# o1-labs/proof-systems

Hardware: AMD Instinct MI355X
Metric: MSM Mscalar/s at 2^20 (Vesta) (higher is better)
Workload: dtype u29x9 / u32x8 (255-bit Montgomery integers); 1 GPU; msm_2^20_vesta_srs; points_per_gpu=1048576, points_total=1048576, bases=SRS::<Vesta>::create, scalars=uniform 254-bit, seed 1234+rank, parallelism=point-range x1, world_size_seen=1

## Files before the change

### include/kimchi_hip.h

```cpp
#ifndef KIMCHI_HIP_H
#define KIMCHI_HIP_H

#include <stddef.h>
#include <stdint.h>

#ifdef __cplusplus
extern "C" {
#endif

#define KH_OK 0
#define KH_E_INVALID (-1)
#define KH_E_DEVICE (-2)
#define KH_E_NOTFOUND (-3)
#define KH_E_NOMEM (-4)

#define KH_CURVE_VESTA 0
#define KH_CURVE_PALLAS 1
#define KH_FIELD_FP 0
#define KH_FIELD_FQ 1
#define KH_BASIS_G (-1)

typedef struct kh_srs kh_srs_t;
typedef struct kh_sponge kh_sponge_t;

// ... 258 lines not shown
int kh_msm_submit_host(kh_srs_t *srs, int basis, unsigned chunk, size_t offset,
                       const uint64_t *scalars , size_t n, size_t k, int scalars_are_montgomery,
                       uint64_t *ticket);
int kh_ntt_dev(int field, uint64_t *data_dev, unsigned log2_n, int inverse, size_t batch);
int kh_lde_dev(int field, const uint64_t *coeffs_dev, unsigned log2_n, unsigned log2_blowup,
               uint64_t *out_dev, size_t batch);
int kh_coset_ntt_dev(int field, const uint64_t *coeffs_dev, unsigned log2_n, const uint64_t shift[4], uint64_t *out_dev, size_t batch);
int kh_sync(void);

int kh_last_timings(const char **names, float *ms, int cap);
uint64_t kh_counter(const char *name);

int kh_debug_field_op(int field, int op, const uint64_t *a, const uint64_t *b, uint64_t *out, size_t n);
int kh_debug_rebase_points(kh_srs_t *srs, const uint64_t *coef, size_t Q, uint64_t *out_xy, uint32_t *out_fail);
int kh_debug_glv_split(int scalar_field, const uint64_t *scalars, size_t n, uint32_t *out);
int kh_debug_point_op(int curve, int op, const uint64_t *p_xy, const uint8_t *p_inf,
                      const uint64_t *q_xy, const uint8_t *q_inf,
                      uint64_t *out_xy, uint8_t *out_inf, size_t n);

typedef struct kh_comm kh_comm_t;
#define KH_COMM_ID_BYTES 128
int kh_comm_unique_id(uint8_t id[128]);
int kh_comm_init(int world_size, int rank, const uint8_t id[128], kh_comm_t **out);
void kh_comm_free(kh_comm_t *comm);
int kh_comm_world_size(const kh_comm_t *comm);
int kh_comm_rank(const kh_comm_t *comm);
int kh_comm_allgather_points(kh_comm_t *comm, const uint64_t *xy, const uint8_t *inf, size_t k, uint64_t *out_xy, uint8_t *out_inf);
int kh_msm_allreduce(kh_comm_t *comm, kh_srs_t *shard, const uint64_t *scalars, size_t n, int scalars_are_montgomery, uint64_t out_xy[8],
                     uint8_t *out_is_inf);

// ... 151 lines not shown
```

### proof_systems_amd/csrc/common.hpp

```cpp
#pragma once
#include <hip/hip_runtime.h>
#include <stdarg.h>
#include <stdint.h>
#include <stdio.h>
#include <atomic>
#include <chrono>
#include <condition_variable>
#include <initializer_list>
#include <map>
#include <memory>
#include <mutex>
#include <set>
#include <string>
#include <thread>
#include <vector>

#include "../../include/kimchi_hip.h"

namespace kh {

void set_error(const char* fmt, ...);

#define KH_HIP(expr)                                                                         \
    do {                                                                                     \
// ... 92 lines not shown
        ws_b29, ws_a1, ws_l2, ws_a2, ws_xlist;
    void* pinned = nullptr; size_t pinned_cap = 0;
    hipEvent_t done = nullptr;
    bool busy = false;
    std::thread::id owner;
    uint64_t ticket = 0;
    MsmJob job;
    std::shared_ptr<std::atomic<int>> handle_jobs;
    volatile uint32_t* host_abort = nullptr;
    volatile uint32_t* spread_abort = nullptr;
    bool flag_unavailable = false;
    bool pinned_coherent = false;
    volatile uint32_t* done_flag = nullptr;
    DevBuf ws_done;
    uint32_t done_expect = 0;
};
static constexpr int MSM_SLOTS = 4;

struct Context {
    std::mutex mu;
    std::condition_variable cv;
    int sync_inflight = 0;
    std::multiset<std::thread::id> blocked_owners;
    int device = -1;
    bool ready = false;
    hipStream_t stream = nullptr;
    bool main_dirty = false;
    hipEvent_t order_ev = nullptr;
    int num_cus = 256;
    size_t lds_per_cu = (size_t)160 << 10, lds_per_block = (size_t)64 << 10;
    bool fused_disabled = false;
    PhaseTimer timer;
    std::vector<std::pair<const char*, float>> last;
    MsmSlot slot[MSM_SLOTS];
    uint64_t next_ticket = 1;
    std::chrono::steady_clock::time_point last_sync_msm_arrival{};
    DevBuf ws_ntt_a, ws_ntt_b;
    void* pinned = nullptr; size_t pinned_cap = 0;
    char* stage = nullptr; size_t stage_cap = 0, stage_cur = 0;
    int stage_upload(void* dst_dev, std::initializer_list<std::pair<const void*, size_t>> parts);
    void mark_async() { if (hipEventRecord(order_ev, stream) == hipSuccess) main_dirty = true; }
    std::mutex scratch_mu;
    std::map<std::string, DevBuf> scratch_bufs;
    std::set<std::string> done_flags;
    DevBuf& scratch(const char* name) { std::lock_guard<std::mutex> lk(scratch_mu); return scratch_bufs[name]; }
    bool once(const char* name) { std::lock_guard<std::mutex> lk(scratch_mu); return done_flags.insert(name).second; }
    void trim_scratch() { std::lock_guard<std::mutex> lk(scratch_mu); for (auto& kv : scratch_bufs) kv.second.release(); }
};
static constexpr int KH_MAX_DEVICES = 16;

// ... 23 lines not shown
```

### proof_systems_amd/csrc/debug_api.cpp

```cpp
#include "api_internal.hpp"

using namespace kh;

extern "C" {

int kh_debug_rebase_points(kh_srs_t* srs, const uint64_t* coef, size_t Q, uint64_t* out_xy, uint32_t* out_fail) {
    KH_ON_DEVICE_OF(srs);
    KH_REQUIRE(srs && coef && out_xy && out_fail, "kh_debug_rebase_points: null argument");
    KH_REQUIRE(srs->g_precomp_c == 16, "the handle has no c = 16 window tables");
    KH_REQUIRE(Q >= 1 && srs->n % Q == 0 && (srs->n / Q) % 64 == 0, "Q = %zu must divide the SRS size %zu into a multiple of 64", Q, srs->n);
    int rc = ensure_init(); if (rc) return rc;
    Context& C = ctx();
    std::lock_guard<std::mutex> lk(C.mu);
    const size_t N = srs->n / Q;
    DevBuf B, part, lists, out, dcoef, fail, scratch;
    if ((rc = B.reserve(rebase_bucket_bytes(N))) || (rc = part.reserve(rebase_part_bytes(N))) || (rc = lists.reserve(rebase_list_bytes(Q))) || (rc = out.reserve(N * 64)) ||
        (rc = dcoef.reserve(Q * 32)) || (rc = fail.reserve(64)) || (rc = scratch.reserve(N * 128))) return rc;
    KH_HIP(hipMemcpyAsync(dcoef.p, coef, Q * 32, hipMemcpyHostToDevice, C.stream));
    KH_HIP(hipMemsetAsync(fail.p, 0, 64, C.stream));
    if ((rc = rebase_points(C.stream, srs->curve, dcoef.as<uint64_t>(), Q, srs->g.p, srs->g_stride, N, B.p, part.p, lists.p))) return rc;
    if ((rc = rebase_tables(C.stream, srs->curve, part.p, N, nullptr, 0, 256, scratch.p, out.p, fail.as<uint32_t>()))) return rc;
    KH_HIP(hipMemcpyAsync(out_xy, out.p, N * 64, hipMemcpyDeviceToHost, C.stream));
    KH_HIP(hipMemcpyAsync(out_fail, fail.p, 4, hipMemcpyDeviceToHost, C.stream));
    KH_HIP(hipStreamSynchronize(C.stream));
    return KH_OK;
}
int kh_debug_glv_split(int scalar_field, const uint64_t* scalars, size_t n, uint32_t* out) {
    KH_REQUIRE(scalar_field == KH_FIELD_FP || scalar_field == KH_FIELD_FQ, "unknown field id %d", scalar_field);
    KH_REQUIRE(scalars && out, "kh_debug_glv_split: null argument");
    int rc = ensure_init(); if (rc) return rc;
    if (n == 0) return KH_OK;
    Context& C = ctx();
    std::lock_guard<std::mutex> lk(C.mu);
    DevBuf din, dout;
    if ((rc = din.reserve(n * 32)) || (rc = dout.reserve(n * 40))) return rc;
    KH_HIP(hipMemcpyAsync(din.p, scalars, n * 32, hipMemcpyHostToDevice, C.stream));
    if ((rc = msm_debug_glv_split(C.stream, scalar_field, din.as<uint64_t>(), n, dout.as<uint32_t>()))) return rc;
    KH_HIP(hipMemcpyAsync(out, dout.p, n * 40, hipMemcpyDeviceToHost, C.stream));
    KH_HIP(hipStreamSynchronize(C.stream));
    return KH_OK;
}
int kh_debug_field_op(int field, int op, const uint64_t* a, const uint64_t* b, uint64_t* out, size_t n) {
    KH_REQUIRE(a && out, "null argument");
    int rc = ensure_init(); if (rc) return rc;
    if (n == 0) return KH_OK;
    Context& C = ctx();
    std::lock_guard<std::mutex> lk(C.mu);
    void *da = nullptr, *db = nullptr, *dout = nullptr;
    KH_HIP(hipMalloc(&da, n * 32)); KH_HIP(hipMalloc(&dout, n * 32));
    KH_HIP(hipMemcpy(da, a, n * 32, hipMemcpyHostToDevice));
    if (b) { KH_HIP(hipMalloc(&db, n * 32)); KH_HIP(hipMemcpy(db, b, n * 32, hipMemcpyHostToDevice)); }
    rc = debug_field_op(C, field, op, (const uint64_t*)da, (const uint64_t*)db, (uint64_t*)dout, n);
    if (rc == KH_OK) { KH_HIP(hipStreamSynchronize(C.stream)); KH_HIP(hipMemcpy(out, dout, n * 32, hipMemcpyDeviceToHost)); }
    (void)hipFree(da); (void)hipFree(dout); if (db) (void)hipFree(db);
// ... 35 lines not shown
```

### proof_systems_amd/csrc/msm.hip

```cpp
#include <hip/hip_ext.h>
#include <math.h>
#include "common.hpp"
#include "env.hpp"
#include "curve.cuh"
#include "coop.cuh"
#include "field29.cuh"
#include "host_ec.hpp"
#include "msm.hpp"
#include <condition_variable>
#include <functional>
#include <memory>
#include <thread>

namespace kh {

#define KH_HIGH_PRIO() __builtin_amdgcn_s_setprio(3)

class HostHelper {
    std::thread th_; std::mutex m_; std::condition_variable cv_, done_cv_;
    std::function<void()> job_; bool has_job_ = false, busy_ = false, stop_ = false;
    void loop() {
        std::unique_lock<std::mutex> lk(m_);
        for (;;) {
            cv_.wait(lk, [&] { return has_job_ || stop_; });
// ... 644 lines not shown
        }
        i += 4 * FUSED_T;
        while (i >= g.n) { i -= g.n; w++; }
    }
    __syncthreads();
    KH_TS(8);
    if (tid == 0) {
        const u32 out = __hip_atomic_fetch_add(sync + 1, 1u, __ATOMIC_RELAXED, __HIP_MEMORY_SCOPE_AGENT);
        if (out == G - 1) {
            __hip_atomic_store(sync, 0u, __ATOMIC_RELAXED, __HIP_MEMORY_SCOPE_AGENT);
            __hip_atomic_store(sync + 1, 0u, __ATOMIC_RELAXED, __HIP_MEMORY_SCOPE_AGENT);
        }
    }
}
static constexpr u32 PART2_MAXLOW = 11, PART2_MAXPASS = 8;
__global__ void __launch_bounds__(PART_T)
k_part2_scatter(const int32_t* __restrict__ digits, u32 tot_e, u32 nblk, u32 low, const u32* __restrict__ PO, u32* __restrict__ mid, u32* __restrict__ xlist, u32* __restrict__ big) {
    KH_HIGH_PRIO();
    __shared__ u32 cur[PART_P];
    const u32 blk = blockIdx.x, j = blockIdx.y, tid = threadIdx.x;
    if (blk == 0 && j == 0 && tid == 0) { xlist[0] = 0; xlist[1] = 0; big[0] = 0; }
    if (tid < PART_P) cur[tid] = PO[((size_t)j * PART_P + tid) * nblk + blk];
    __syncthreads();
    const u32 e_lo = (u32)((u64)tot_e * blk / nblk), e_hi = (u32)((u64)tot_e * (blk + 1) / nblk);
    const int32_t* d = digits + (size_t)j * tot_e;
    for (u32 e0 = e_lo + tid; e0 < e_hi; e0 += 8 * PART_T) {
        int32_t v[8];
#pragma unroll
        for (int u = 0; u < 8; u++) { const u32 e = e0 + u * PART_T; v[u] = d[e < e_hi ? e : e_hi - 1]; if (e >= e_hi) v[u] = 0; }
#pragma unroll
        for (int u = 0; u < 8; u++) {
            const u32 b = (u32)(v[u] < 0 ? -v[u] : v[u]) - 1u;
            const u32 pos = lds_inc_agg(cur, b & (PART_P - 1u), v[u] != 0);
            if (v[u]) mid[pos] = ((b >> 8) << 17) | (v[u] < 0 ? 1u << 16 : 0u) | (e0 + u * PART_T - e_lo);
        }
    }
}
struct WideTasks { u32 room, kmin, nkeys; KTab ktab; };
__global__ void __launch_bounds__(PART_T)
k_part2_sort(const u32* __restrict__ mid, const u32* __restrict__ PO, u32 nblk, u32 low, u32 nb, u32 tot_e, u32 n, size_t pt_stride, size_t pt_offset,
             size_t pt_batch, u32 last_group, size_t total_idx, WideTasks ta, u32* __restrict__ off, u32* __restrict__ entries,
             u32* __restrict__ toff, u32* __restrict__ order, u32* __restrict__ ptot, u32* __restrict__ xlist, u32* __restrict__ slist,
             uint8_t* __restrict__ buckets29, u32 og, u32 stage_cap, u32 max_pass, u32* __restrict__ big, u32 bigcap, u32 hot_nt) {
    KH_HIGH_PRIO();
    __shared__ u32 cur[1u << PART2_MAXLOW], pstart[1025], bi0[1024], bw0[1024], lh[MAX_K + 2], sh[PART_T / 64 + 1];
    __shared__ u32 xl_n, pfirst[PART2_MAXPASS], plast[PART2_MAXPASS];
    extern __shared__ u32 stage[];
    u32* const xl_key = stage; u32* const xl_nt = stage + (1u << PART2_MAXLOW); u32* const xl_base = stage + (2u << PART2_MAXLOW);
    const u32 pidx = blockIdx.x, j = blockIdx.y, tid = threadIdx.x;
    const size_t q = (size_t)j * PART_P + pidx;
    const u32 nparts = gridDim.x * gridDim.y;
    const u32 nbl = 1u << low;
    for (u32 i = tid; i <= nblk; i += PART_T) pstart[i] = PO[q * nblk + i];
    for (u32 i = tid; i < nblk; i += PART_T) {
        const u32 est = (u32)((u64)tot_e * i / nblk), w0 = est / n;
        bw0[i] = w0; bi0[i] = est - w0 * n;
    }
    for (u32 i = tid; i < nbl; i += PART_T) cur[i] = 0;
    for (u32 i = tid; i < MAX_K + 2; i += PART_T) lh[i] = 0;
    if (tid == 0) xl_n = 0;
    __syncthreads();
    const u32 base = pstart[0], end = pstart[nblk];
    for (u32 x0 = base + tid; x0 < end; x0 += 8 * PART_T) {
        u32 m[8];
#pragma unroll
        for (int u = 0; u < 8; u++) { const u32 x = x0 + u * PART_T; m[u] = mid[x < end ? x : end - 1]; }
#pragma unroll
        for (int u = 0; u < 8; u++) (void)lds_inc_agg(cur, m[u] >> 17, x0 + u * PART_T < end);
    }
    __syncthreads();
    {
        const u32 i0 = 2 * tid, a = i0 < nbl ? cur[i0] : 0u, b = i0 + 1 < nbl ? cur[i0 + 1] : 0u;
        u32 btot;
        const u32 ex = base + block_scan_1024(a + b, sh, &btot);
        __syncthreads();
        const size_t key0 = (size_t)j * nb + (size_t)pidx * nbl + i0;
        if (i0 < nbl) { off[key0] = ex; cur[i0] = ex; }
        if (i0 + 1 < nbl) { off[key0 + 1] = ex + a; cur[i0 + 1] = ex + a; }
        if (tid == 0 && pidx == PART_P - 1 && j == last_group) off[(size_t)(j + 1) * nb] = end;
        const u32 K = pick_K(PO[total_idx], ta.room, ta.kmin, ta.ktab, ta.nkeys);
        const u32 nta = (a + K - 1) / K, ntb = (b + K - 1) / K;
        const u32 la = nta ? (a + nta - 1) / nta : 0u, lb = ntb ? (b + ntb - 1) / ntb : 0u;
        const u32 tex = block_scan_1024(nta + ntb, sh, &btot);
        if (i0 < nbl) toff[key0] = tex;
        if (i0 + 1 < nbl) toff[key0 + 1] = tex + nta;
        if (tid == 0) ptot[q] = btot;
        if (i0 < nbl) atomicAdd(&lh[la], 1u);
        if (i0 + 1 < nbl) atomicAdd(&lh[lb], 1u);
        if (nta > 1) { const u32 sl = atomicAdd(&xl_n, 1u); xl_key[sl] = (u32)key0; xl_nt[sl] = nta; xl_base[sl] = atomicAdd(&xlist[0], nta - 1u); slist[atomicAdd(&xlist[1], 1u)] = (u32)key0; }
        if (ntb > 1) { const u32 sl = atomicAdd(&xl_n, 1u); xl_key[sl] = (u32)key0 + 1u; xl_nt[sl] = ntb; xl_base[sl] = atomicAdd(&xlist[0], ntb - 1u); slist[atomicAdd(&xlist[1], 1u)] = (u32)key0 + 1u; }
        if (nta > hot_nt) { const u32 sl = atomicAdd(&big[0], 1u); big[2 + sl] = (u32)key0; big[2 + bigcap + sl] = 0u; }
        if (ntb > hot_nt) { const u32 sl = atomicAdd(&big[0], 1u); big[2 + sl] = (u32)key0 + 1u; big[2 + bigcap + sl] = 0u; }
        if (i0 < nbl && a == 0) { uint4* rec = (uint4*)(buckets29 + ((size_t)j * nb + ((size_t)i0 << 8 | pidx)) * B29_BYTES); _Pragma("unroll") for (int t = 0; t < 9; t++) rec[t] = make_uint4(0u, 0u, 0u, 0u); }
        if (i0 + 1 < nbl && b == 0) { uint4* rec = (uint4*)(buckets29 + ((size_t)j * nb + ((size_t)(i0 + 1) << 8 | pidx)) * B29_BYTES); _Pragma("unroll") for (int t = 0; t < 9; t++) rec[t] = make_uint4(0u, 0u, 0u, 0u); }
        __syncthreads();
        const u32 L = MAX_K - (tid <= MAX_K ? tid : MAX_K), hv = tid <= MAX_K ? lh[L] : 0u;
        const u32 above = block_scan_1024(hv, sh, &btot);
        __syncthreads();
        if (tid <= MAX_K) lh[L] = above;
        __syncthreads();
        if (i0 < nbl) { const u32 r = atomicAdd(&lh[la], 1u); order[(size_t)(r / og) * nparts * og + q * og + (r % og)] = (u32)key0; }
        if (i0 + 1 < nbl) { const u32 r = atomicAdd(&lh[lb], 1u); order[(size_t)(r / og) * nparts * og + q * og + (r % og)] = (u32)key0 + 1u; }
        const u32 nx = xl_n;
        for (u32 it = 0; it < nx; it++) {
            const u32 key = xl_key[it], ntx = xl_nt[it], xb = xl_base[it];
            for (u32 jt = 1 + tid; jt < ntx; jt += PART_T) { xlist[2 + 2 * (size_t)(xb + jt - 1)] = key; xlist[3 + 2 * (size_t)(xb + jt - 1)] = jt; }
        }
    }
    __syncthreads();
    const u32 pb0 = (u32)(pt_offset + (size_t)j * pt_batch);
    const u32 lane = tid & 63u, wv = tid >> 6;
    const u32 S_eff = stage_cap > 2048u ? stage_cap - 1024u : 0u;
    const u32 npass = S_eff ? (end - base + S_eff - 1u) / S_eff : 0u;
    const bool staged = S_eff != 0u && npass >= 1u && npass <= max_pass;
    uint8_t* const bpass = (uint8_t*)(stage + stage_cap);
    if (staged) {
        if (tid < PART2_MAXPASS) { pfirst[tid] = 0xffffffffu; plast[tid] = 0u; }
// ... 28 lines not shown
                        if (staged && pos - p0 < stage_cap) stage[pos - p0] = val;
                        else entries[pos] = val;
                    }
                }
            }
        }
        if (staged) {
            __syncthreads();
            const u32 cnt = p1 - p0 < stage_cap ? p1 - p0 : stage_cap;
            for (u32 k = tid; k < cnt; k += PART_T) entries[p0 + k] = stage[k];
            __syncthreads();
        }
    }
}
__global__ void __launch_bounds__(256)
k_wide_fixup(u32* __restrict__ toff, const u32* __restrict__ ptot, u32 nparts, u32 low, u32 nkeys, u32* __restrict__ handed, u32* __restrict__ big) {
    KH_HIGH_PRIO();
    __shared__ u32 sh[4];
    const u32 key = blockIdx.x * 256 + threadIdx.x, q = (blockIdx.x * 256) >> low;
    u32 v = 0;
    for (u32 t = threadIdx.x; t < q && t < nparts; t += 256) v += ptot[t];
#pragma unroll
    for (int d = 32; d >= 1; d >>= 1) v += __shfl_xor(v, d, 64);
    if ((threadIdx.x & 63u) == 0) sh[threadIdx.x >> 6] = v;
    __syncthreads();
    const u32 bs = sh[0] + sh[1] + sh[2] + sh[3];
    if (key < nkeys) toff[key] += bs;
    else if (key == nkeys) toff[key] = bs;
    if (key == 0) handed[0] = 0;
}
template <class BF>
__global__ void __launch_bounds__(256) __attribute__((amdgpu_num_vgpr(112), amdgpu_waves_per_eu(4, 4)))
k_accumulate29(const u32* __restrict__ entries, const u32* __restrict__ off, const u32* __restrict__ toff,
               const u32* __restrict__ roff, const u32* __restrict__ order,
// ... 729 lines not shown
            const double len = std::min<double>(K, m + 2.3 * sqrt(m));
            const double cost = ceil(blocks / cus) * len + 2.0 * tpb;
            if (cost < best - 1e-9) { best = cost; bk = K; }
        }
        t.k[idx] = (uint8_t)bk;
    }
    cache[{nkeys, cus}] = t;
    return t;
}

template <class CFG>
static int msm_enqueue_t(Context& Ctx, MsmSlot& C, const MsmBasis& basis, size_t offset, const u64* scalars_dev, size_t n, size_t k,
                         int mont, int curve, int flags) {
    typedef typename CFG::Base BF; typedef typename CFG::Scalar SF;
    hipStream_t s = C.stream;
    const bool wide = basis.wide_pts && basis.wide_c > 16 && basis.wide_c - 9 <= (int)PART2_MAXLOW && n >= msm_wide_min_n() && k <= 4 &&
                      (size_t)windows_of(basis.wide_c) * n <= ((size_t)1 << 26);
    static constexpr u32 SPREAD_MAX_NT = 256;
    const void* const tab_pts = wide ? basis.wide_pts : basis.pts;
    const int c = wide ? basis.wide_c : (basis.precomp_c ? basis.precomp_c : msm_pick_window(n));
    const bool glv = basis.glv && !wide && basis.precomp_c != 0;
    const int W = glv ? 2 * ((128 + c - 1) / c) : windows_of(c);
    const u32 nb = 1u << (c - 1);
    const int precomp = (wide || basis.precomp_c) ? 1 : 0;
    int S = (int)(n / 32768); if (S < 1) S = 1; if (S > 16) S = 16;
    { int want = (int)(512 / ((size_t)W * k)); if (want < 1) want = 1; if (S > want) S = want; }
    const size_t tab_stride = basis.stride ? basis.stride : basis.n;
    SortGeom g{n, nb, S, W, precomp, tab_stride, offset, basis.batch_stride};
    const size_t ngroups = precomp ? k : k * (size_t)W;
    const bool few_groups = ngroups <= 8;
// ... 13 lines not shown

    int rc;
    if ((rc = C.ws_digits.reserve(M * sizeof(int32_t)))) return rc;
    if ((rc = C.ws_hist.reserve(nkeys * Sq * sizeof(u32)))) return rc;
    if ((rc = C.ws_cnt.reserve((nkeys + 2) * sizeof(u32)))) return rc;
    if ((rc = C.ws_off.reserve((nkeys + 2) * sizeof(u32)))) return rc;
    if ((rc = C.ws_ntask.reserve((nkeys + 2) * sizeof(u32)))) return rc;
    if ((rc = C.ws_toff.reserve((nkeys + 2) * sizeof(u32)))) return rc;
    if ((rc = C.ws_entries.reserve((M + 1) * sizeof(u32)))) return rc;
    if ((rc = C.ws_partial.reserve(max_tasks * 128))) return rc;
    if ((rc = C.ws_handed.reserve((max_tasks + 2) * sizeof(u32)))) return rc;
    if ((rc = C.ws_buckets.reserve(nkeys * 128))) return rc;
    const size_t bigcap = nkeys + max_tasks / CHUNK + 2;
    if ((rc = C.ws_biglist.reserve((2 + 4 * bigcap) * sizeof(u32)))) return rc;
    if ((rc = C.ws_chunks.reserve(bigcap * 128))) return rc;
    if ((rc = C.ws_order.reserve((2 * (MAX_K + 1) + 3 * (nkeys + 2)) * sizeof(u32)))) return rc;
    WideGeom wg{};
    static constexpr u32 wide_og = 16, wide_acc_blocks = 3, wide_rlog = 4;
    static_assert((wide_og & (wide_og - 1)) == 0 && wide_og <= (1u << (17 - 9)) && wide_rlog >= 1 && wide_rlog + 2 <= 17 / 2, "wide-path constants");
    size_t wide_acc_lds = (Ctx.lds_per_cu / (wide_acc_blocks + 1) + 1024) & ~(size_t)1023;
    if (wide_acc_lds > Ctx.lds_per_block) wide_acc_lds = Ctx.lds_per_block & ~(size_t)1023;
    if (wide) {
        if ((rc = C.ws_xlist.reserve((3 * max_tasks + 8) * sizeof(u32)))) return rc;
        if ((rc = C.ws_handed.reserve((2 * max_tasks + 4) * sizeof(u32)))) return rc;
        wg.nb = nb; wg.lo = (u32)c / 2; wg.hi = (u32)(c - 1) - wg.lo; wg.rlog = wide_rlog;
        wg.flog = wg.lo > wg.rlog + 5 ? wg.lo - wg.rlog - 4 : 1;
        if ((rc = C.ws_b29.reserve(nkeys * B29_BYTES))) return rc;
        if ((rc = C.ws_a1.reserve(ngroups * 2 * (size_t)(nb >> wg.rlog) * B29_BYTES))) return rc;
        if ((rc = C.ws_l2.reserve(ngroups * 2 * (size_t)(nb >> (wg.rlog + wg.flog)) * B29_BYTES))) return rc;
        if ((rc = C.ws_a2.reserve(ngroups * 2 * ((size_t)1 << wg.lo) * 128))) return rc;
    }
    u32 m = 1;
    while (m < 16 && (ngroups * (size_t)nb) / m > 65536) m <<= 1;
    if (!precomp && m < 4) m = 4;
// ... 75 lines not shown
        }
    }
    C.timer.begin(s);
    if (glv)
    hipLaunchKernelGGL((k_digits_glv<SF>), dim3((unsigned)((n + 255) / 256), (unsigned)k), dim3(256), 0, s,
                       scalars_dev, basis.inf, offset, basis.batch_stride, n, mont, c, W, C.ws_digits.as<int32_t>());
    else
    hipLaunchKernelGGL((k_digits<SF>), dim3((unsigned)((n + 255) / 256), (unsigned)k), dim3(256), 0, s,
                       scalars_dev, basis.inf, offset, basis.batch_stride, n, mont, c, W, C.ws_digits.as<int32_t>(), (size_t)0, n);
    C.timer.mark("digits", s);
    u32* len_hist = C.ws_order.as<u32>();
    u32* cursor = len_hist + (MAX_K + 1);
    u32* order = cursor + (MAX_K + 1);
    u32* rnt = order + (nkeys + 2);
    u32* roff = rnt + (nkeys + 2);
    if (fused) {
        order = nullptr; roff = C.ws_toff.as<u32>();
        u32* sy = C.ws_sync.as<u32>();
        hipLaunchKernelGGL(k_sort_fused, dim3(fg.bpg * fg.k * fg.split), dim3(FUSED_T), (size_t)fg.sub * sizeof(u32), s, C.ws_digits.as<int32_t>(), fg,
                           C.ws_hist.as<u32>(), C.ws_off.as<u32>(), C.ws_toff.as<u32>(), C.ws_entries.as<u32>(), C.ws_handed.as<u32>(),
                           C.ws_biglist.as<u32>(), sy, sy + 2, C.host_abort, fused_spin_ticks);
        C.timer.mark("sort", s);
    } else if (part) {
        const u32 tot_e = (u32)((size_t)W * n);
        const dim3 pgrid(part_nblk, (unsigned)k);
        hipLaunchKernelGGL(k_part_hist, pgrid, dim3(PART_T), 0, s, C.ws_digits.as<int32_t>(), tot_e, part_nblk, wide ? 0u : part_low, C.ws_hist.as<u32>());
        C.timer.mark("histogram", s);
        if ((rc = exclusive_scan_u32(C.ws_hist.as<u32>(), C.ws_cnt.as<u32>(), part_size + 1, C.ws_scan_tmp, s))) return rc;
        C.timer.mark("scan", s);
        if (wide) {
            hipLaunchKernelGGL(k_part2_scatter, pgrid, dim3(PART_T), 0, s, C.ws_digits.as<int32_t>(), tot_e, part_nblk, part_low, C.ws_cnt.as<u32>(), C.ws_mid.as<u32>(), C.ws_xlist.as<u32>(), C.ws_biglist.as<u32>());
            const WideTasks wt{room, kmin, (u32)nkeys, ktab};
            u32* const slist = C.ws_xlist.as<u32>() + 2 + 2 * max_tasks;
            u32* const ptot = C.ws_ntask.as<u32>();
            const u32 part2_stage = sort_staging_cell(0).load(), part2_maxpass = std::min<u32>(PART2_MAXPASS, sort_staging_cell(1).load());
            u32 stage_now = std::min<u32>(part2_stage, (131072u - (1u << PART2_MAXLOW)) / 4u);
            if (stage_now <= 2048u || (size_t)W * n / PART_P > (size_t)part2_maxpass * (stage_now - 1024u)) stage_now = 0;
            const u32 stage_words = std::max<u32>(stage_now, 3u << PART2_MAXLOW);
            const size_t part2_lds = (size_t)stage_words * 4 + (stage_now ? ((size_t)1 << PART2_MAXLOW) : 0);
            if (Ctx.once("part2_attr")) KH_HIP(hipFuncSetAttribute((const void*)k_part2_sort, hipFuncAttributeMaxDynamicSharedMemorySize, 131072));
            hipLaunchKernelGGL(k_part2_sort, dim3(PART_P, (unsigned)k), dim3(PART_T), part2_lds, s, C.ws_mid.as<u32>(), C.ws_cnt.as<u32>(), part_nblk, part_low, nb, tot_e, (u32)n,
                               tab_stride, offset, basis.batch_stride, (u32)(k - 1), part_size, wt, C.ws_off.as<u32>(), C.ws_entries.as<u32>(),
                               C.ws_toff.as<u32>(), order, ptot, C.ws_xlist.as<u32>(), slist, C.ws_b29.as<uint8_t>(), wide_og, stage_now, part2_maxpass, C.ws_biglist.as<u32>(), (u32)bigcap, WIDE_HOT_NT);
            hipLaunchKernelGGL(k_wide_fixup, dim3((unsigned)(nkeys / 256 + 1)), dim3(256), 0, s, C.ws_toff.as<u32>(), ptot, (u32)(k * PART_P), part_low, (u32)nkeys,
                               C.ws_handed.as<u32>(), C.ws_biglist.as<u32>());
        } else {
        hipLaunchKernelGGL(k_part_scatter, pgrid, dim3(PART_T), 0, s, C.ws_digits.as<int32_t>(), tot_e, (u32)n, part_nblk, C.ws_cnt.as<u32>(), C.ws_mid.as<u32>());
        hipLaunchKernelGGL(k_part_sort, dim3(PART_P, (unsigned)k), dim3(PART_T), 0, s, C.ws_mid.as<u32>(), C.ws_cnt.as<u32>(), part_nblk, nb,
                           tab_stride, offset, basis.batch_stride, (u32)(k - 1), C.ws_off.as<u32>(), C.ws_entries.as<u32>());
        }
        C.timer.mark("scatter", s);
    } else {
        size_t lds = (size_t)nb * sizeof(u32);
        dim3 sgrid((unsigned)S, (unsigned)W, (unsigned)k);
        hipLaunchKernelGGL(k_hist, sgrid, dim3(1024), lds, s, C.ws_digits.as<int32_t>(), g, C.ws_hist.as<u32>());
        hipLaunchKernelGGL(k_key_totals, dim3((unsigned)((nkeys + 1 + 255) / 256)), dim3(256), 0, s,
                           C.ws_hist.as<u32>(), nb, Sq, nkeys, C.ws_cnt.as<u32>());
        C.timer.mark("histogram", s);
        if ((rc = exclusive_scan_u32(C.ws_cnt.as<u32>(), C.ws_off.as<u32>(), nkeys + 1, C.ws_scan_tmp, s))) return rc;
        C.timer.mark("scan", s);
// ... 325 lines not shown
```

### proof_systems_amd/csrc/msm_api.cpp

```cpp
#include <stdlib.h>
#include <algorithm>
#include <chrono>

#include "api_internal.hpp"
#include "env.hpp"

using namespace kh;

static int free_slot(Context& C) {
    for (int i = 0; i < MSM_SLOTS; i++) if (!C.slot[i].busy) return i;
    return -1;
}
int kh::acquire_slot(std::unique_lock<std::mutex>* lk, Context& C, bool side_first) {
    const auto me = std::this_thread::get_id();
    auto t_start = std::chrono::steady_clock::now();
    uint64_t seen = ~(uint64_t)0;
    for (;;) {
        uint64_t sig = C.next_ticket;
        for (int i = 0; i < MSM_SLOTS; i++) sig = sig * 1315423911ull + (C.slot[i].busy ? C.slot[i].ticket + 1 : 0);
        if (sig != seen) { seen = sig; t_start = std::chrono::steady_clock::now(); }
        int si = -1;
        if (side_first) for (int i = MSM_SLOTS - 1; i >= 1; i--) if (!C.slot[i].busy) { si = i; break; }
        if (si < 0) si = free_slot(C);
        if (si >= 0 || !lk) return si;
// ... 75 lines not shown
            }
            e = hipEventQuery(ev);
            if (e != hipErrorNotReady) break;
            if (std::chrono::duration_cast<std::chrono::microseconds>(std::chrono::steady_clock::now() - t0).count() > spin_us) break;
            __builtin_ia32_pause();
        }
    }
    if (e == hipErrorNotReady) { (void)hipGetLastError(); e = hipEventSynchronize(ev); }
    tl_last_wait_us = std::chrono::duration<double, std::micro>(std::chrono::steady_clock::now() - tw0).count();
    lk.lock();
    C.sync_inflight--;
    if (by_flag && !flag_seen && e == hipSuccess) S.done_expect = __atomic_load_n((const uint32_t*)S.done_flag, __ATOMIC_ACQUIRE);
    int rc;
    if (e != hipSuccess) { set_error("hipEventSynchronize: %s", hipGetErrorString(e)); S.busy = false; rc = KH_E_DEVICE; }
    else rc = msm_finish(C, S, out_xy, out_inf, flag_seen);
    uncount_handle_job(S);
    C.cv.notify_all();
    return rc;
}
struct CoalesceMember { const uint64_t* scalars; uint64_t* out_xy; uint8_t* out_inf; };
struct CoalesceGroup {
    kh_srs_t* srs; int basis; unsigned chunk; size_t offset, n; int mont;
    std::vector<CoalesceMember> members;
    bool closed = false, done = false;
    int rc = KH_OK;
    std::string err;
    std::condition_variable cv;
};
static constexpr size_t COALESCE_MAX = 32;
static std::vector<std::shared_ptr<CoalesceGroup>>& coalesce_groups(Context& C) {
// ... 308 lines not shown
```

### proof_systems_amd/khip.py

```python
from __future__ import annotations

import ctypes as C
import os

import numpy as np

from . import _abi

_HERE = os.path.dirname(os.path.abspath(__file__))
LIB_PATH = os.environ.get("KH_LIB") or os.path.join(_HERE, "libkimchi_hip.so")

if not os.path.exists(LIB_PATH):
    raise ImportError(f"{LIB_PATH} is missing: run `python -c 'import __graft_entry__ as g; g.build()'` "
                      "(hipcc --offload-arch=gfx950); there is no CPU fallback")
try:
    _PROTOTYPES, _STRUCTS, _CONSTANTS = _abi.parse()
except OSError as e:
    raise ImportError(f"{_abi.HEADER} is missing: the binding is declared from it ({e})") from e

_lib = C.CDLL(LIB_PATH)

SYMBOLS = list(_PROTOTYPES)

def __getattr__(name: str):
# ... 116 lines not shown

def set_sort_staging(entries: int = 28672, max_passes: int = 2):
    _check(_lib.kh_msm_set_sort_staging(entries, max_passes))


def glv_split(scalar_field: int, scalars):
    a = np.ascontiguousarray(scalars, dtype=np.uint64)
    n = a.shape[0]
    out = np.zeros((n, 10), np.uint32)
    _check(_lib.kh_debug_glv_split(scalar_field, _p64(a), n, out.ctypes.data_as(C.POINTER(C.c_uint32))))
    res = []
    for row in out:
        m1 = sum(int(row[t]) << (32 * t) for t in range(4)); m2 = sum(int(row[4 + t]) << (32 * t) for t in range(4))
        res.append((-m1 if row[8] else m1, -m2 if row[9] else m2))
    return res


def set_wide_min_n(n: int):
    _check(_lib.kh_msm_set_wide_min_n(n))


class Srs:

    def __init__(self, curve: int, g_xy=None, depth: int = 0, start: int = 0):
        self.curve = curve
        self._h = C.c_void_p()
        if g_xy is None:
            self.n = depth
            _check(_lib.kh_srs_create_device_range(curve, start, depth, C.byref(self._h)))
        else:
# ... 1266 lines not shown
```

### rust/kimchi-hip-sys/src/lib.rs

```rust
#![allow(non_camel_case_types, clippy::too_many_arguments, clippy::missing_safety_doc)]

use core::ffi::{c_char, c_int, c_uint, c_void};

#[repr(C)]
pub struct kh_srs_t {
    _private: [u8; 0],
}
#[repr(C)]
pub struct kh_ipa_t {
    _private: [u8; 0],
}
#[repr(C)]
pub struct kh_sponge_t {
    _private: [u8; 0],
}
#[repr(C)]
pub struct kh_prover_index_t {
    _private: [u8; 0],
}
#[repr(C)]
pub struct kh_proof_t {
    _private: [u8; 0],
}
#[repr(C)]
// ... 313 lines not shown
    pub fn kh_dev_upload_2d(dst_dev: *mut c_void, dst_pitch: usize, src_host: *const c_void, src_pitch: usize, width: usize, rows: usize) -> c_int;
    pub fn kh_dev_upload_2d_unordered(dst_dev: *mut c_void, dst_pitch: usize, src_host: *const c_void, src_pitch: usize, width: usize, rows: usize) -> c_int;
    pub fn kh_msm_batch_dev(srs: *mut kh_srs_t, basis: c_int, chunk: c_uint, offset: usize, scalars_dev: *const u64, n: usize, k: usize, scalars_are_montgomery: c_int, out_xy: *mut u64, out_is_inf: *mut u8) -> c_int;
    pub fn kh_msm_submit(srs: *mut kh_srs_t, basis: c_int, chunk: c_uint, offset: usize, scalars_dev: *const u64, n: usize, k: usize, scalars_are_montgomery: c_int, ticket: *mut u64) -> c_int;
    pub fn kh_msm_wait(ticket: u64, out_xy: *mut u64, out_is_inf: *mut u8) -> c_int;
    pub fn kh_msm_submit_host(srs: *mut kh_srs_t, basis: c_int, chunk: c_uint, offset: usize, scalars: *const u64, n: usize, k: usize, scalars_are_montgomery: c_int, ticket: *mut u64) -> c_int;
    pub fn kh_ntt_dev(field: c_int, data_dev: *mut u64, log2_n: c_uint, inverse: c_int, batch: usize) -> c_int;
    pub fn kh_lde_dev(field: c_int, coeffs_dev: *const u64, log2_n: c_uint, log2_blowup: c_uint, out_dev: *mut u64, batch: usize) -> c_int;
    pub fn kh_coset_ntt_dev(field: c_int, coeffs_dev: *const u64, log2_n: c_uint, shift: *const u64, out_dev: *mut u64, batch: usize) -> c_int;
    pub fn kh_sync() -> c_int;
    pub fn kh_last_timings(names: *mut *const c_char, ms: *mut f32, cap: c_int) -> c_int;
    pub fn kh_counter(name: *const c_char) -> u64;
    pub fn kh_debug_field_op(field: c_int, op: c_int, a: *const u64, b: *const u64, out: *mut u64, n: usize) -> c_int;
    pub fn kh_debug_rebase_points(srs: *mut kh_srs_t, coef: *const u64, Q: usize, out_xy: *mut u64, out_fail: *mut u32) -> c_int;
    pub fn kh_debug_glv_split(scalar_field: c_int, scalars: *const u64, n: usize, out: *mut u32) -> c_int;
    pub fn kh_debug_point_op(curve: c_int, op: c_int, p_xy: *const u64, p_inf: *const u8, q_xy: *const u64, q_inf: *const u8, out_xy: *mut u64, out_inf: *mut u8, n: usize) -> c_int;
    pub fn kh_comm_unique_id(id: *mut u8) -> c_int;
    pub fn kh_comm_init(world_size: c_int, rank: c_int, id: *const u8, out: *mut *mut kh_comm_t) -> c_int;
    pub fn kh_comm_free(comm: *mut kh_comm_t);
    pub fn kh_comm_world_size(comm: *const kh_comm_t) -> c_int;
    pub fn kh_comm_rank(comm: *const kh_comm_t) -> c_int;
    pub fn kh_comm_allgather_points(comm: *mut kh_comm_t, xy: *const u64, inf: *const u8, k: usize, out_xy: *mut u64, out_inf: *mut u8) -> c_int;
    pub fn kh_msm_allreduce(comm: *mut kh_comm_t, shard: *mut kh_srs_t, scalars: *const u64, n: usize, scalars_are_montgomery: c_int, out_xy: *mut u64, out_is_inf: *mut u8) -> c_int;
    pub fn kh_lookup_sorted(table: *const u64, lookup_rows: usize, values: *const u64, value_stride: usize, max_per_row: usize, out: *mut u64, bad_row: *mut usize) -> c_int;
    pub fn kh_lookup_sorted_dev(table_dev: *const u64, lookup_rows: usize, values_dev: *const u64, value_stride: usize, max_per_row: usize, out_dev: *mut u64, out_stride: usize, bad_row: *mut usize) -> c_int;
    pub fn kh_prover_index_new(srs: *mut kh_srs_t, log2_n: c_uint, zk_rows: c_uint, public_inputs: c_uint, d1_dev: *const u64, dc_dev: *const u64, d8_dev: *const u64, optional_gates: *const c_int, n_optional: usize, live_mask: c_uint, shifts: *const u64, digest: *const u64, out: *mut *mut kh_prover_index_t) -> c_int;
    pub fn kh_prover_index_attach_lookup(index: *mut kh_prover_index_t, patterns: *const c_int, n_patterns: usize, selectors_d1_dev: *const *const u64, selectors_c_dev: *const *const u64, selectors_d8_dev: *const *const u64, table_cols_d1_dev: *const *const u64, n_table_cols: usize, table_ids_d1_dev: *const u64, atoms_d8_dev: *const *const u64) -> c_int;
    pub fn kh_prover_index_attach_runtime_tables(index: *mut kh_prover_index_t, selector_d1_dev: *const u64, selector_c_dev: *const u64, selector_d8_dev: *const u64, offset: usize, length: usize) -> c_int;
    pub fn kh_permutation_shifts(field: c_int, log2_n: c_uint, out: *mut u64) -> c_int;
    pub fn kh_prover_index_create(srs: *mut kh_srs_t, n_gates: usize, gate_types: *const c_int, wires: *const u32, coeffs: *const u64, public_inputs: c_uint, out: *mut *mut kh_prover_index_t) -> c_int;
// ... 37 lines not shown
```

Baseline: 1099 Mscalar/s.

## Build a globally level-sorted bucket order for the wide MSM path

Replaces the interleaved per-partition bucket ordering (groups of 16 per partition per round) with a global counting sort by level. Each partition records per-key level and rank, writes per-level counts to a cell table, and a new k_wide_cells kernel prefix-scans those counts across levels and partitions. k_wide_fixup then scatters each key to its global slot. This gives downstream accumulation a strictly level-ordered work list, at the cost of an extra kernel launch and extra workspace. A debug API exposing the plan is also added.

```diff
diff --git a/include/kimchi_hip.h b/include/kimchi_hip.h
--- a/include/kimchi_hip.h
+++ b/include/kimchi_hip.h
@@ -296,6 +296,7 @@
 int kh_debug_field_op(int field, int op, const uint64_t *a, const uint64_t *b, uint64_t *out, size_t n);
 int kh_debug_rebase_points(kh_srs_t *srs, const uint64_t *coef, size_t Q, uint64_t *out_xy, uint32_t *out_fail);
 int kh_debug_glv_split(int scalar_field, const uint64_t *scalars, size_t n, uint32_t *out);
+int kh_debug_wide_plan(uint32_t *order, uint32_t *off, uint32_t *toff, size_t cap, size_t *nkeys, unsigned *low);
 int kh_debug_point_op(int curve, int op, const uint64_t *p_xy, const uint8_t *p_inf,
                       const uint64_t *q_xy, const uint8_t *q_inf,
                       uint64_t *out_xy, uint8_t *out_inf, size_t n);
diff --git a/proof_systems_amd/csrc/common.hpp b/proof_systems_amd/csrc/common.hpp
--- a/proof_systems_amd/csrc/common.hpp
+++ b/proof_systems_amd/csrc/common.hpp
@@ -130,6 +130,7 @@
     volatile uint32_t* done_flag = nullptr;
     DevBuf ws_done;
     uint32_t done_expect = 0;
+    const uint32_t* wide_order = nullptr; size_t wide_nkeys = 0; unsigned wide_low = 0;
 };
 static constexpr int MSM_SLOTS = 4;
 
@@ -150,6 +151,7 @@
     std::vector<std::pair<const char*, float>> last;
     MsmSlot slot[MSM_SLOTS];
     uint64_t next_ticket = 1;
+    int last_wide_slot = -1; uint64_t last_wide_ticket = 0;
     std::chrono::steady_clock::time_point last_sync_msm_arrival{};
     DevBuf ws_ntt_a, ws_ntt_b;
     void* pinned = nullptr; size_t pinned_cap = 0;
diff --git a/proof_systems_amd/csrc/debug_api.cpp b/proof_systems_amd/csrc/debug_api.cpp
--- a/proof_systems_amd/csrc/debug_api.cpp
+++ b/proof_systems_amd/csrc/debug_api.cpp
@@ -38,6 +38,25 @@
     if ((rc = msm_debug_glv_split(C.stream, scalar_field, din.as<uint64_t>(), n, dout.as<uint32_t>()))) return rc;
     KH_HIP(hipMemcpyAsync(out, dout.p, n * 40, hipMemcpyDeviceToHost, C.stream));
     KH_HIP(hipStreamSynchronize(C.stream));
+    return KH_OK;
+}
+int kh_debug_wide_plan(uint32_t* order, uint32_t* off, uint32_t* toff, size_t cap, size_t* nkeys, unsigned* low) {
+    KH_REQUIRE(nkeys && low, "kh_debug_wide_plan: null argument");
+    int rc = ensure_init(); if (rc) return rc;
+    Context& C = ctx();
+    std::lock_guard<std::mutex> lk(C.mu);
+    const int si = C.last_wide_slot;
+    if (si < 0 || C.slot[si].busy || !C.slot[si].wide_order || C.slot[si].ticket != C.last_wide_ticket) {
+        set_error("kh_debug_wide_plan: no wide MSM whose plan is still in its slot's workspace"); return KH_E_NOTFOUND;
+    }
+    MsmSlot& S = C.slot[si];
+    *nkeys = S.wide_nkeys; *low = S.wide_low;
+    if (cap <= S.wide_nkeys) return KH_OK;
+    KH_REQUIRE(order && off && toff, "kh_debug_wide_plan: null argument");
+    KH_HIP(hipStreamSynchronize(S.stream));
+    KH_HIP(hipMemcpy(order, S.wide_order, S.wide_nkeys * sizeof(uint32_t), hipMemcpyDeviceToHost));
+    KH_HIP(hipMemcpy(off, S.ws_off.p, (S.wide_nkeys + 1) * sizeof(uint32_t), hipMemcpyDeviceToHost));
+    KH_HIP(hipMemcpy(toff, S.ws_toff.p, (S.wide_nkeys + 1) * sizeof(uint32_t), hipMemcpyDeviceToHost));
     return KH_OK;
 }
 int kh_debug_field_op(int field, int op, const uint64_t* a, const uint64_t* b, uint64_t* out, size_t n) {
diff --git a/proof_systems_amd/csrc/msm.hip b/proof_systems_amd/csrc/msm.hip
--- a/proof_systems_amd/csrc/msm.hip
+++ b/proof_systems_amd/csrc/msm.hip
@@ -682,12 +682,22 @@
     }
 }
 static constexpr u32 PART2_MAXLOW = 11, PART2_MAXPASS = 8;
+static constexpr u32 WIDE_NL = MAX_K + 2;
+struct WidePlan {
+    static constexpr size_t HEAD = 2 * (MAX_K + 1);
+    static size_t words(size_t nkeys, size_t nparts) { return HEAD + 3 * (nkeys + 2) + (size_t)WIDE_NL * nparts; }
+    __host__ __device__ static u32* rowtot(u32* order) { return order - HEAD; }
+    __host__ __device__ static u32* rankw(u32* order, size_t nkeys) { return order + (nkeys + 2); }
+    __host__ __device__ static u32* cells(u32* order, size_t nkeys) { return order + 3 * (nkeys + 2); }
+};
 __global__ void __launch_bounds__(PART_T)
-k_part2_scatter(const int32_t* __restrict__ digits, u32 tot_e, u32 nblk, u32 low, const u32* __restrict__ PO, u32* __restrict__ mid, u32* __restrict__ xlist, u32* __restrict__ big) {
+k_part2_scatter(const int32_t* __restrict__ digits, u32 tot_e, u32 nblk, u32 low, const u32* __restrict__ PO, u32* __restrict__ mid, u32* __restrict__ xlist, u32* __restrict__ big,
+                u32* __restrict__ rowtot) {
     KH_HIGH_PRIO();
     __shared__ u32 cur[PART_P];
     const u32 blk = blockIdx.x, j = blockIdx.y, tid = threadIdx.x;
     if (blk == 0 && j == 0 && tid == 0) { xlist[0] = 0; xlist[1] = 0; big[0] = 0; }
+    if (blk == 0 && j == 0 && tid < WIDE_NL) rowtot[tid] = 0;
     if (tid < PART_P) cur[tid] = PO[((size_t)j * PART_P + tid) * nblk + blk];
     __syncthreads();
     const u32 e_lo = (u32)((u64)tot_e * blk / nblk), e_hi = (u32)((u64)tot_e * (blk + 1) / nblk);
@@ -709,9 +719,9 @@
 k_part2_sort(const u32* __restrict__ mid, const u32* __restrict__ PO, u32 nblk, u32 low, u32 nb, u32 tot_e, u32 n, size_t pt_stride, size_t pt_offset,
              size_t pt_batch, u32 last_group, size_t total_idx, WideTasks ta, u32* __restrict__ off, u32* __restrict__ entries,
              u32* __restrict__ toff, u32* __restrict__ order, u32* __restrict__ ptot, u32* __restrict__ xlist, u32* __restrict__ slist,
-             uint8_t* __restrict__ buckets29, u32 og, u32 stage_cap, u32 max_pass, u32* __restrict__ big, u32 bigcap, u32 hot_nt) {
-    KH_HIGH_PRIO();
-    __shared__ u32 cur[1u << PART2_MAXLOW], pstart[1025], bi0[1024], bw0[1024], lh[MAX_K + 2], sh[PART_T / 64 + 1];
+             uint8_t* __restrict__ buckets29, u32 stage_cap, u32 max_pass, u32* __restrict__ big, u32 bigcap, u32 hot_nt) {
+    KH_HIGH_PRIO();
+    __shared__ u32 cur[1u << PART2_MAXLOW], pstart[1025], bi0[1024], bw0[1024], lh[WIDE_NL], sh[PART_T / 64 + 1];
     __shared__ u32 xl_n, pfirst[PART2_MAXPASS], plast[PART2_MAXPASS];
     extern __shared__ u32 stage[];
     u32* const xl_key = stage; u32* const xl_nt = stage + (1u << PART2_MAXLOW); u32* const xl_base = stage + (2u << PART2_MAXLOW);
@@ -719,13 +729,14 @@
     const size_t q = (size_t)j * PART_P + pidx;
     const u32 nparts = gridDim.x * gridDim.y;
     const u32 nbl = 1u << low;
+    u32* const rowtot = WidePlan::rowtot(order); u32* const rankw = WidePlan::rankw(order, ta.nkeys); u32* const cells = WidePlan::cells(order, ta.nkeys);
     for (u32 i = tid; i <= nblk; i += PART_T) pstart[i] = PO[q * nblk + i];
     for (u32 i = tid; i < nblk; i += PART_T) {
         const u32 est = (u32)((u64)tot_e * i / nblk), w0 = est / n;
         bw0[i] = w0; bi0[i] = est - w0 * n;
     }
     for (u32 i = tid; i < nbl; i += PART_T) cur[i] = 0;
-    for (u32 i = tid; i < MAX_K + 2; i += PART_T) lh[i] = 0;
+    for (u32 i = tid; i < WIDE_NL; i += PART_T) lh[i] = 0;
     if (tid == 0) xl_n = 0;
     __syncthreads();
     const u32 base = pstart[0], end = pstart[nblk];
@@ -753,8 +764,8 @@
         if (i0 < nbl) toff[key0] = tex;
         if (i0 + 1 < nbl) toff[key0 + 1] = tex + nta;
         if (tid == 0) ptot[q] = btot;
-        if (i0 < nbl) atomicAdd(&lh[la], 1u);
-        if (i0 + 1 < nbl) atomicAdd(&lh[lb], 1u);
+        if (i0 < nbl) rankw[key0] = la << 16 | atomicAdd(&lh[la], 1u);
+        if (i0 + 1 < nbl) rankw[key0 + 1] = lb << 16 | atomicAdd(&lh[lb], 1u);
         if (nta > 1) { const u32 sl = atomicAdd(&xl_n, 1u); xl_key[sl] = (u32)key0; xl_nt[sl] = nta; xl_base[sl] = atomicAdd(&xlist[0], nta - 1u); slist[atomicAdd(&xlist[1], 1u)] = (u32)key0; }
         if (ntb > 1) { const u32 sl = atomicAdd(&xl_n, 1u); xl_key[sl] = (u32)key0 + 1u; xl_nt[sl] = ntb; xl_base[sl] = atomicAdd(&xlist[0], ntb - 1u); slist[atomicAdd(&xlist[1], 1u)] = (u32)key0 + 1u; }
         if (nta > hot_nt) { const u32 sl = atomicAdd(&big[0], 1u); big[2 + sl] = (u32)key0; big[2 + bigcap + sl] = 0u; }
@@ -762,13 +773,7 @@
         if (i0 < nbl && a == 0) { uint4* rec = (uint4*)(buckets29 + ((size_t)j * nb + ((size_t)i0 << 8 | pidx)) * B29_BYTES); _Pragma("unroll") for (int t = 0; t < 9; t++) rec[t] = make_uint4(0u, 0u, 0u, 0u); }
         if (i0 + 1 < nbl && b == 0) { uint4* rec = (uint4*)(buckets29 + ((size_t)j * nb + ((size_t)(i0 + 1) << 8 | pidx)) * B29_BYTES); _Pragma("unroll") for (int t = 0; t < 9; t++) rec[t] = make_uint4(0u, 0u, 0u, 0u); }
         __syncthreads();
-        const u32 L = MAX_K - (tid <= MAX_K ? tid : MAX_K), hv = tid <= MAX_K ? lh[L] : 0u;
-        const u32 above = block_scan_1024(hv, sh, &btot);
-        __syncthreads();
-        if (tid <= MAX_K) lh[L] = above;
-        __syncthreads();
-        if (i0 < nbl) { const u32 r = atomicAdd(&lh[la], 1u); order[(size_t)(r / og) * nparts * og + q * og + (r % og)] = (u32)key0; }
-        if (i0 + 1 < nbl) { const u32 r = atomicAdd(&lh[lb], 1u); order[(size_t)(r / og) * nparts * og + q * og + (r % og)] = (u32)key0 + 1u; }
+        if (tid < WIDE_NL) { const u32 c = lh[tid], row = WIDE_NL - 1u - tid; cells[(size_t)row * nparts + q] = c; if (c) atomicAdd(&rowtot[row], c); }
         const u32 nx = xl_n;
         for (u32 it = 0; it < nx; it++) {
             const u32 key = xl_key[it], ntx = xl_nt[it], xb = xl_base[it];
@@ -827,10 +832,44 @@
     }
 }
 __global__ void __launch_bounds__(256)
-k_wide_fixup(u32* __restrict__ toff, const u32* __restrict__ ptot, u32 nparts, u32 low, u32 nkeys, u32* __restrict__ handed, u32* __restrict__ big) {
+k_wide_cells(u32* __restrict__ cells, const u32* __restrict__ rowtot, u32 nparts) {
+    KH_HIGH_PRIO();
+    __shared__ u32 sh[8];
+    const u32 row = blockIdx.x, tid = threadIdx.x, lane = tid & 63u, wave = tid >> 6;
+    if (rowtot[row] == 0u) return;
+    u32 v = 0;
+    for (u32 t = tid; t < row; t += 256) v += rowtot[t];
+#pragma unroll
+    for (int d = 32; d >= 1; d >>= 1) v += __shfl_xor(v, d, 64);
+    if (lane == 0) sh[wave] = v;
+    __syncthreads();
+    u32 carry = sh[0] + sh[1] + sh[2] + sh[3];
+    u32* const rowp = cells + (size_t)row * nparts;
+    for (u32 q0 = 0; q0 < nparts; q0 += 256) {
+        const u32 c = rowp[q0 + tid];
+        u32 inc = c;
+#pragma unroll
+        for (int d = 1; d < 64; d <<= 1) { const u32 o = __shfl_up(inc, d, 64); if (lane >= (u32)d) inc += o; }
+        if (lane == 63) sh[4 + wave] = inc;
+        __syncthreads();
+        u32 below = 0, tot = 0;
+#pragma unroll
+        for (u32 w = 0; w < 4; w++) { const u32 t = sh[4 + w]; if (w < wave) below += t; tot += t; }
+        rowp[q0 + tid] = carry + below + inc - c;
+        carry += tot;
+        __syncthreads();
+    }
+}
+__global__ void __launch_bounds__(256)
+k_wide_fixup(u32* __restrict__ toff, const u32* __restrict__ ptot, u32 nparts, u32 low, u32 nkeys, u32* __restrict__ handed, u32* __restrict__ big,
+             const u32* __restrict__ rankw, const u32* __restrict__ cells, u32* __restrict__ order) {
     KH_HIGH_PRIO();
     __shared__ u32 sh[4];
     const u32 key = blockIdx.x * 256 + threadIdx.x, q = (blockIdx.x * 256) >> low;
+    if (key < nkeys) {
+        const u32 w = rankw[key], L = w >> 16, slot = cells[(size_t)(WIDE_NL - 1u - (L < WIDE_NL ? L : 0u)) * nparts + q] + (w & 0xffffu);
+        if (slot < nkeys) order[slot] = key;
+    }
     u32 v = 0;
     for (u32 t = threadIdx.x; t < q && t < nparts; t += 256) v += ptot[t];
 #pragma unroll
@@ -1590,6 +1629,7 @@
                          int mont, int curve, int flags) {
     typedef typename CFG::Base BF; typedef typename CFG::Scalar SF;
     hipStream_t s = C.stream;
+    C.wide_order = nullptr;
     const bool wide = basis.wide_pts && basis.wide_c > 16 && basis.wide_c - 9 <= (int)PART2_MAXLOW && n >= msm_wide_min_n() && k <= 4 &&
                       (size_t)windows_of(basis.wide_c) * n <= ((size_t)1 << 26);
     static constexpr u32 SPREAD_MAX_NT = 256;
@@ -1633,10 +1673,10 @@
     const size_t bigcap = nkeys + max_tasks / CHUNK + 2;
     if ((rc = C.ws_biglist.reserve((2 + 4 * bigcap) * sizeof(u32)))) return rc;
     if ((rc = C.ws_chunks.reserve(bigcap * 128))) return rc;
-    if ((rc = C.ws_order.reserve((2 * (MAX_K + 1) + 3 * (nkeys + 2)) * sizeof(u32)))) return rc;
+    if ((rc = C.ws_order.reserve(WidePlan::words(nkeys, wide ? PART_P * k : 0) * sizeof(u32)))) return rc;
     WideGeom wg{};
-    static constexpr u32 wide_og = 16, wide_acc_blocks = 3, wide_rlog = 4;
-    static_assert((wide_og & (wide_og - 1)) == 0 && wide_og <= (1u << (17 - 9)) && wide_rlog >= 1 && wide_rlog + 2 <= 17 / 2, "wide-path constants");
+    static constexpr u32 wide_acc_blocks = 3, wide_rlog = 4;
+    static_assert(wide_rlog >= 1 && wide_rlog + 2 <= 17 / 2 && WIDE_NL <= 2 * (MAX_K + 1) && PART2_MAXLOW <= 16, "wide-path constants");
     size_t wide_acc_lds = (Ctx.lds_per_cu / (wide_acc_blocks + 1) + 1024) & ~(size_t)1023;
     if (wide_acc_lds > Ctx.lds_per_block) wide_acc_lds = Ctx.lds_per_block & ~(size_t)1023;
     if (wide) {
@@ -1742,6 +1782,7 @@
     u32* order = cursor + (MAX_K + 1);
     u32* rnt = order + (nkeys + 2);
     u32* roff = rnt + (nkeys + 2);
+    u32* const wide_rowtot = WidePlan::rowtot(order); u32* const wide_rankw = WidePlan::rankw(order, nkeys); u32* const wide_cells = WidePlan::cells(order, nkeys);
     if (fused) {
         order = nullptr; roff = C.ws_toff.as<u32>();
         u32* sy = C.ws_sync.as<u32>();
@@ -1757,7 +1798,7 @@
         if ((rc = exclusive_scan_u32(C.ws_hist.as<u32>(), C.ws_cnt.as<u32>(), part_size + 1, C.ws_scan_tmp, s))) return rc;
         C.timer.mark("scan", s);
         if (wide) {
-            hipLaunchKernelGGL(k_part2_scatter, pgrid, dim3(PART_T), 0, s, C.ws_digits.as<int32_t>(), tot_e, part_nblk, part_low, C.ws_cnt.as<u32>(), C.ws_mid.as<u32>(), C.ws_xlist.as<u32>(), C.ws_biglist.as<u32>());
+            hipLaunchKernelGGL(k_part2_scatter, pgrid, dim3(PART_T), 0, s, C.ws_digits.as<int32_t>(), tot_e, part_nblk, part_low, C.ws_cnt.as<u32>(), C.ws_mid.as<u32>(), C.ws_xlist.as<u32>(), C.ws_biglist.as<u32>(), wide_rowtot);
             const WideTasks wt{room, kmin, (u32)nkeys, ktab};
             u32* const slist = C.ws_xlist.as<u32>() + 2 + 2 * max_tasks;
             u32* const ptot = C.ws_ntask.as<u32>();
@@ -1769,9 +1810,12 @@
             if (Ctx.once("part2_attr")) KH_HIP(hipFuncSetAttribute((const void*)k_part2_sort, hipFuncAttributeMaxDynamicSharedMemorySize, 131072));
             hipLaunchKernelGGL(k_part2_sort, dim3(PART_P, (unsigned)k), dim3(PART_T), part2_lds, s, C.ws_mid.as<u32>(), C.ws_cnt.as<u32>(), part_nblk, part_low, nb, tot_e, (u32)n,
                                tab_stride, offset, basis.batch_stride, (u32)(k - 1), part_size, wt, C.ws_off.as<u32>(), C.ws_entries.as<u32>(),
-                               C.ws_toff.as<u32>(), order, ptot, C.ws_xlist.as<u32>(), slist, C.ws_b29.as<uint8_t>(), wide_og, stage_now, part2_maxpass, C.ws_biglist.as<u32>(), (u32)bigcap, WIDE_HOT_NT);
+                               C.ws_toff.as<u32>(), order, ptot, C.ws_xlist.as<u32>(), slist, C.ws_b29.as<uint8_t>(), stage_now, part2_maxpass,
+                               C.ws_biglist.as<u32>(), (u32)bigcap, WIDE_HOT_NT);
+            hipLaunchKernelGGL(k_wide_cells, dim3(WIDE_NL), dim3(256), 0, s, wide_cells, wide_rowtot, (u32)(k * PART_P));
             hipLaunchKernelGGL(k_wide_fixup, dim3((unsigned)(nkeys / 256 + 1)), dim3(256), 0, s, C.ws_toff.as<u32>(), ptot, (u32)(k * PART_P), part_low, (u32)nkeys,
-                               C.ws_handed.as<u32>(), C.ws_biglist.as<u32>());
+                               C.ws_handed.as<u32>(), C.ws_biglist.as<u32>(), wide_rankw, wide_cells, order);
+            C.wide_order = order; C.wide_nkeys = nkeys; C.wide_low = part_low;
         } else {
         hipLaunchKernelGGL(k_part_scatter, pgrid, dim3(PART_T), 0, s, C.ws_digits.as<int32_t>(), tot_e, (u32)n, part_nblk, C.ws_cnt.as<u32>(), C.ws_mid.as<u32>());
         hipLaunchKernelGGL(k_part_sort, dim3(PART_P, (unsigned)k), dim3(PART_T), 0, s, C.ws_mid.as<u32>(), C.ws_cnt.as<u32>(), part_nblk, nb,
diff --git a/proof_systems_amd/csrc/msm_api.cpp b/proof_systems_amd/csrc/msm_api.cpp
--- a/proof_systems_amd/csrc/msm_api.cpp
+++ b/proof_systems_amd/csrc/msm_api.cpp
@@ -113,6 +113,7 @@
     int rc;
     if (e != hipSuccess) { set_error("hipEventSynchronize: %s", hipGetErrorString(e)); S.busy = false; rc = KH_E_DEVICE; }
     else rc = msm_finish(C, S, out_xy, out_inf, flag_seen);
+    if (rc == KH_OK && S.wide_order) { C.last_wide_slot = (int)(&S - C.slot); C.last_wide_ticket = S.ticket; }
     uncount_handle_job(S);
     C.cv.notify_all();
     return rc;
diff --git a/proof_systems_amd/khip.py b/proof_systems_amd/khip.py
--- a/proof_systems_amd/khip.py
+++ b/proof_systems_amd/khip.py
@@ -154,6 +154,16 @@
         m1 = sum(int(row[t]) << (32 * t) for t in range(4)); m2 = sum(int(row[4 + t]) << (32 * t) for t in range(4))
         res.append((-m1 if row[8] else m1, -m2 if row[9] else m2))
     return res
+
+
+def wide_plan():
+    nkeys, low = C.c_size_t(), C.c_uint()
+    _check(_lib.kh_debug_wide_plan(None, None, None, 0, C.byref(nkeys), C.byref(low)))
+    n = nkeys.value
+    order, off, toff = np.zeros(n, np.uint32), np.zeros(n + 1, np.uint32), np.zeros(n + 1, np.uint32)
+    p32 = lambda a: a.ctypes.data_as(C.POINTER(C.c_uint32))
+    _check(_lib.kh_debug_wide_plan(p32(order), p32(off), p32(toff), n + 1, C.byref(nkeys), C.byref(low)))
+    return order, off, toff, low.value
 
 
 def set_wide_min_n(n: int):
diff --git a/rust/kimchi-hip-sys/src/lib.rs b/rust/kimchi-hip-sys/src/lib.rs
--- a/rust/kimchi-hip-sys/src/lib.rs
+++ b/rust/kimchi-hip-sys/src/lib.rs
@@ -351,6 +351,7 @@
     pub fn kh_debug_field_op(field: c_int, op: c_int, a: *const u64, b: *const u64, out: *mut u64, n: usize) -> c_int;
     pub fn kh_debug_rebase_points(srs: *mut kh_srs_t, coef: *const u64, Q: usize, out_xy: *mut u64, out_fail: *mut u32) -> c_int;
     pub fn kh_debug_glv_split(scalar_field: c_int, scalars: *const u64, n: usize, out: *mut u32) -> c_int;
+    pub fn kh_debug_wide_plan(order: *mut u32, off: *mut u32, toff: *mut u32, cap: usize, nkeys: *mut usize, low: *mut c_uint) -> c_int;
     pub fn kh_debug_point_op(curve: c_int, op: c_int, p_xy: *const u64, p_inf: *const u8, q_xy: *const u64, q_inf: *const u8, out_xy: *mut u64, out_inf: *mut u8, n: usize) -> c_int;
     pub fn kh_comm_unique_id(id: *mut u8) -> c_int;
     pub fn kh_comm_init(world_size: c_int, rank: c_int, id: *const u8, out: *mut *mut kh_comm_t) -> c_int;
```

Result: no change. 1098 Mscalar/s (-0.1%).
